# danielreardon/scintools

Measured on AMD Instinct MI355X. Metric: eta_curvature_sweep_points_per_sec, higher is better.
Workload: dtype f64

## Files before the change

scintools_amd/csrc/eigen_packed.hip:

```cpp
#include <math.h>
#include <string.h>

#include <algorithm>
#include <atomic>
#include <map>
#include <vector>

#include "packed.hpp"
#include "prof.hpp"

namespace scint {

constexpr int kCheckEveryBlock = 2;
constexpr int kFirstCheck = 8;
constexpr int kMaxK = 512;

__device__ inline cplx packed_at(const PackedJob& jb, int r, int c) {
    const int br = r / kTB, bc = c / kTB;
    if (bc >= br) return jb.tiles[(tile_offset(jb.nb, br) + (bc - br)) * kTileElems + (r % kTB) * kTB + (c % kTB)];
    return conj(jb.tiles[(tile_offset(jb.nb, bc) + (br - bc)) * kTileElems + (c % kTB) * kTB + (r % kTB)]);
}

constexpr int kRedGroups = 4;


__global__ void __launch_bounds__(64) pk_ritz_scale_kernel(const PackedJob* jobs, const int32_t* slots,
                                                           const int64_t* eta_index, cplx* vec_out,
                                                           int64_t vstride) {
    const PackedJob jb = jobs[slots[blockIdx.y]];
    const int K = blockIdx.x, e = threadIdx.x;
    if (K >= jb.nb) return;
    double t = 0.0;
    for (int i = e; i < jb.nb; i += 64) t += jb.upart[0][i];
    t = wave_sum(t);
    const double inv = t > 0.0 ? 1.0 / sqrt(t) : 0.0;
    const int r = K * kTB + e;
    cplx* out = vec_out + eta_index[blockIdx.y] * vstride;
    if (r < jb.n) out[r] = mk(out[r].x * inv, out[r].y * inv);
}

struct Blk2 {
    double a11, a22; cplx a12;
    double b11, b22; cplx b12;
    double i11, i22;
};

__device__ inline Blk2 step_block_wave(const double* __restrict__ ap, const double* __restrict__ up, int nb, int lane,
                                       bool direct = false) {
    double s[8];
#pragma unroll
    for (int c = 0; c < 8; ++c) s[c] = 0.0;
    for (int i = lane; i < nb; i += 64) {
#pragma unroll
        for (int c = 0; c < 4; ++c) { s[c] += gload(ap + 4 * i + c); s[4 + c] += gload(up + 4 * i + c); }
    }
#pragma unroll
    for (int c = 0; c < 8; ++c) s[c] = wave_sum(s[c]);
    Blk2 b;
    b.a11 = s[0]; b.a22 = s[1]; b.a12 = mk(s[2], s[3]);
    const double n12 = s[2] * s[2] + s[3] * s[3], tr = s[0] + s[1];
    const double h11 = direct ? s[4] : s[4] - (s[0] * s[0] + n12), h22 = direct ? s[5] : s[5] - (n12 + s[1] * s[1]);
    const cplx h12 = direct ? mk(s[6], s[7]) : mk(s[6] - s[2] * tr, s[7] - s[3] * tr);
    const double kPivotFloor = direct ? 0.0 : 1e-14;
    b.b11 = h11 > kPivotFloor * s[4] ? sqrt(h11) : 0.0;
    b.i11 = b.b11 > 0.0 ? 1.0 / b.b11 : 0.0;
    b.b12 = mk(h12.x * b.i11, h12.y * b.i11);
    const double d = h22 - norm2(b.b12);
    b.b22 = d > kPivotFloor * s[5] ? sqrt(d) : 0.0;
    b.i22 = b.b22 > 0.0 ? 1.0 / b.b22 : 0.0;
    return b;
}

__device__ inline void blk_q_row(const Blk2& b, cplx u1, cplx u2, cplx q1, cplx q2, cplx& x1, cplx& x2) {
    const cplx y1 = u1 - (q1 * b.a11 + mulc(q2, b.a12));
    const cplx y2 = u2 - (q1 * b.a12 + q2 * b.a22);
    x1 = y1 * b.i11;
    x2 = (y2 - x1 * b.b12) * b.i22;
}

__device__ inline int second_start_row(int n) { return (n / 2 + 7 < n) ? n / 2 + 7 : (n / 2 + 1) % max(n, 1); }

__global__ void __launch_bounds__(64) pk2_init_kernel(const PackedJob* jobs, const int32_t* slots) {
    const PackedJob jb = jobs[slots[blockIdx.y]];
    const int K = blockIdx.x, e = threadIdx.x;
    if (K == 0 && e == 0) { jb.state[1] = 0; jb.result[1] = -INFINITY; jb.result[3] = -INFINITY; }
    if (K >= jb.nb) return;
    const int r = K * kTB + e;
    cplx v0 = mk(0.0, 0.0), v1 = mk(0.0, 0.0);
    if (r < jb.n && jb.n >= 2) { v0 = packed_at(jb, jb.n / 2, r); v1 = packed_at(jb, second_start_row(jb.n), r); }
    jb.U[0][2 * r] = v0; jb.U[0][2 * r + 1] = v1;
    jb.U[1][2 * r] = mk(0.0, 0.0); jb.U[1][2 * r + 1] = mk(0.0, 0.0);
    cplx* qm1 = jb.Q + (int64_t)(jb.qslots - 1) * jb.qstride * 2;
    qm1[2 * r] = mk(0.0, 0.0); qm1[2 * r + 1] = mk(0.0, 0.0);
    jb.Q[2 * r] = mk(0.0, 0.0); jb.Q[2 * r + 1] = mk(0.0, 0.0);
    const double g11 = wave_sum(norm2(v0)), g22 = wave_sum(norm2(v1));
    const cplx g12 = wave_sum(mulc(v1, v0));
    if (e == 0) {
#pragma unroll
        for (int c = 0; c < 4; ++c) { jb.apart[0][4 * K + c] = 0.0; jb.apart[1][4 * K + c] = 0.0; jb.upart[1][4 * K + c] = 0.0; }
        jb.upart[0][4 * K] = g11; jb.upart[0][4 * K + 1] = g22; jb.upart[0][4 * K + 2] = g12.x; jb.upart[0][4 * K + 3] = g12.y;
    }
}

__device__ inline Blk2 load_blk(const double* __restrict__ c) {
    Blk2 b;
    b.a11 = gload(c + 0); b.a22 = gload(c + 1); b.a12 = mk(gload(c + 2), gload(c + 3));
    b.b11 = gload(c + 4); b.b22 = gload(c + 5); b.b12 = mk(gload(c + 6), gload(c + 7));
    b.i11 = gload(c + 8); b.i22 = gload(c + 9);
    return b;
}

constexpr int kCoefRows = 1024;
__global__ void __launch_bounds__(kCoefRows) pk2_coef_kernel(const PackedJob* __restrict__ jobs, int launch) {
    __shared__ double sh[16];
    const PackedJob jb = jobs[blockIdx.y];
    const int step = launch - jb.start;
    if (jb.n < 2 || step < 0 || step >= jb.max_steps || gload(jb.state) >= jb.gen) return;
    if ((int)blockIdx.x * kCoefRows >= jb.nb * kTB) return;
    const int par = step & 1;
    if (threadIdx.x < 64) {
        const Blk2 sc = step_block_wave(par ? jb.apart[1] : jb.apart[0], par ? jb.upart[1] : jb.upart[0], jb.nb, threadIdx.x,
                                        jb.certify && step == 1);
        if (threadIdx.x == 0) {
            sh[0] = sc.a11; sh[1] = sc.a22; sh[2] = sc.a12.x; sh[3] = sc.a12.y;
            sh[4] = sc.b11; sh[5] = sc.b22; sh[6] = sc.b12.x; sh[7] = sc.b12.y;
            sh[8] = sc.i11; sh[9] = sc.i22;
            if (blockIdx.x == 0) {
                double* c = jb.coef + 16 * par;
#pragma unroll
                for (int i = 0; i < 10; ++i) gstore(c + i, sh[i]);
                if (step > 0) {
                    double* A = jb.alpha + 4 * (step - 1);
                    A[0] = sc.a11; A[1] = sc.a22; A[2] = sc.a12.x; A[3] = sc.a12.y;
                }
                double* B = jb.beta + 4 * step;
                B[0] = sc.b11; B[1] = sc.b22; B[2] = sc.b12.x; B[3] = sc.b12.y;
            }
        }
    }
    __syncthreads();
    Blk2 sc;
    sc.a11 = sh[0]; sc.a22 = sh[1]; sc.a12 = mk(sh[2], sh[3]);
    sc.b11 = sh[4]; sc.b22 = sh[5]; sc.b12 = mk(sh[6], sh[7]);
    sc.i11 = sh[8]; sc.i22 = sh[9];
    const int r = (int)blockIdx.x * kCoefRows + (int)threadIdx.x;
    if (r >= jb.nb * kTB) return;
    const cplx* __restrict__ Up = par ? jb.U[1] : jb.U[0];
    const int qs = jb.qslots;
    const cplx* __restrict__ Qp = jb.Q + (int64_t)((step + qs - 1) % qs) * jb.qstride * 2;
    cplx* __restrict__ Qn = jb.Q + (int64_t)(step % qs) * jb.qstride * 2;
    cplx x1, x2;
    blk_q_row(sc, gload(Up + 2 * r), gload(Up + 2 * r + 1), gload(Qp + 2 * r), gload(Qp + 2 * r + 1), x1, x2);
    gstore(Qn + 2 * r, x1); gstore(Qn + 2 * r + 1, x2);
}

constexpr int kLdsXs = 0, kLdsCol = kMaxStrip * kTB * 2, kLdsXi = 2 * kLdsCol, kLdsRsum = kLdsXi + kRows64 * kTB * 2,
              kLdsElems = kLdsRsum + 4 * kTB * 2;
constexpr size_t kMatvecLdsBytes = sizeof(cplx) * kLdsElems;
static_assert(kMatvecLdsBytes <= 80 * 1024, "two mat-vec workgroups per CU (160 KiB of LDS)");

__device__ __forceinline__ void pk2_half(const cplx (&a)[8], int h, const cplx (*__restrict__ xir)[2],
                                        const cplx (&xJ1)[2], const cplx (&xJ2)[2], cplx (&acc1)[8], cplx (&acc2)[8],
                                        cplx (&c1)[2], cplx (&c2)[2]) {
#pragma unroll
    for (int jj = 0; jj < 4; ++jj) {
        const int j = 4 * h + jj;
        const cplx x1 = xir[8 * j][0], x2 = xir[8 * j][1];
#pragma unroll
        for (int cc = 0; cc < 2; ++cc) {
            const cplx e = a[2 * jj + cc];
            acc1[j] = acc1[j] + e * xJ1[cc];
            acc2[j] = acc2[j] + e * xJ2[cc];
            c1[cc] = mk(c1[cc].x + e.x * x1.x + e.y * x1.y, c1[cc].y + e.x * x1.y - e.y * x1.x);
            c2[cc] = mk(c2[cc].x + e.x * x2.x + e.y * x2.y, c2[cc].y + e.x * x2.y - e.y * x2.x);
        }
// ... 134 lines not shown

__global__ void __launch_bounds__(256, 2)
pk2_matvec_kernel(const Strip* __restrict__ strips, int launch) {
    pk2_matvec_body(strips + blockIdx.x, launch);
}

}
#include "matvec32.hpp"
namespace scint {

__global__ void __launch_bounds__(64 * kRedGroups)
pk2_reduce_kernel(const PackedJob* __restrict__ jobs, int launch) {
    __shared__ cplx part[kRedGroups][kTB][2];
    const PackedJob jb = jobs[blockIdx.y];
    const int K = blockIdx.x;
    const int step = launch - jb.start;
    if (K >= jb.nb || jb.n < 2 || step < 0 || step >= jb.max_steps || gload(jb.state) >= jb.gen) return;
    const int par = step & 1;
    const int g = threadIdx.x >> 6, e = threadIdx.x & 63;
    const int s0 = jb.row_strip0[K], nrow = jb.row_strip0[K + 1] - s0;
    cplx acc1 = mk(0.0, 0.0), acc2 = mk(0.0, 0.0);
    const int lg = jb.rowgroup_lg;
    const int npair = (K + (1 << lg) - 1) >> lg;
    for (int idx = g; idx < nrow + npair; idx += kRedGroups) {
        const int cI = (idx - nrow) << lg;
        const cplx* src = idx < nrow ? jb.rowpart + 2 * ((int64_t)(s0 + idx) * kTB + e)
                                     : jb.colpart + 2 * ((tile_offset(jb.nb, cI) + (K - cI)) * kTB + e);
        acc1 = acc1 + gload(src);
        acc2 = acc2 + gload(src + 1);
    }
    part[g][e][0] = acc1;
    part[g][e][1] = acc2;
    __syncthreads();
    if (g == 0) {
        const Blk2 sc = load_blk(jb.coef + 16 * par);
        cplx tot1 = part[0][e][0], tot2 = part[0][e][1];
#pragma unroll
        for (int k = 1; k < kRedGroups; ++k) { tot1 = tot1 + part[k][e][0]; tot2 = tot2 + part[k][e][1]; }
        const int r = K * kTB + e;
        const cplx* __restrict__ Qp = jb.Q + (int64_t)((step + jb.qslots - 1) % jb.qslots) * jb.qstride * 2;
        const cplx* __restrict__ Qn = jb.Q + (int64_t)(step % jb.qslots) * jb.qstride * 2;
        cplx* __restrict__ Un = par ? jb.U[0] : jb.U[1];
        const cplx q1 = gload(Qp + 2 * r), q2 = gload(Qp + 2 * r + 1);
        const cplx x1 = gload(Qn + 2 * r), x2 = gload(Qn + 2 * r + 1);
        const cplx t1 = tot1 - (q1 * sc.b11 + mulc(q2, sc.b12));
        const cplx t2 = tot2 - q2 * sc.b22;
        gstore(Un + 2 * r, t1); gstore(Un + 2 * r + 1, t2);
        const double pa11 = wave_sum(x1.x * t1.x + x1.y * t1.y);
        const double pa22 = wave_sum(x2.x * t2.x + x2.y * t2.y);
        const cplx pa12 = wave_sum(mulc(t2, x1));
        const double pg11 = wave_sum(norm2(t1)), pg22 = wave_sum(norm2(t2));
        const cplx pg12 = wave_sum(mulc(t2, t1));
        if (e == 0) {
            double* an = par ? jb.apart[0] : jb.apart[1];
            double* un = par ? jb.upart[0] : jb.upart[1];
            an[4 * K] = pa11; an[4 * K + 1] = pa22; an[4 * K + 2] = pa12.x; an[4 * K + 3] = pa12.y;
            un[4 * K] = pg11; un[4 * K + 1] = pg22; un[4 * K + 2] = pg12.x; un[4 * K + 3] = pg12.y;
        }
    }
}

__global__ void __launch_bounds__(64) pk2_cert_resid_kernel(const PackedJob* __restrict__ jobs, int launch) {
    const PackedJob jb = jobs[blockIdx.y];
    const int K = blockIdx.x, e = threadIdx.x;
    if (!jb.certify || launch - jb.start != 0 || K >= jb.nb || jb.n < 2 || gload(jb.state) >= jb.gen) return;
    const Blk2 sc = step_block_wave(jb.apart[1], jb.upart[1], jb.nb, e);
    const int r = K * kTB + e;
    const cplx* __restrict__ Q0 = jb.Q;
    const cplx u1 = gload(jb.U[1] + 2 * r), u2 = gload(jb.U[1] + 2 * r + 1);
    const cplx q1 = gload(Q0 + 2 * r), q2 = gload(Q0 + 2 * r + 1);
    const cplx y1 = u1 - (q1 * sc.a11 + mulc(q2, sc.a12));
    const cplx y2 = u2 - (q1 * sc.a12 + q2 * sc.a22);
    const double g11 = wave_sum(norm2(y1)), g22 = wave_sum(norm2(y2));
    const cplx g12 = wave_sum(mulc(y2, y1));
    if (e == 0) { double* un = jb.upart[1]; un[4 * K] = g11; un[4 * K + 1] = g22; un[4 * K + 2] = g12.x; un[4 * K + 3] = g12.y; }
}

constexpr int kMaxKB = 128;
constexpr int kSvecStride = 2 * kMaxKB + 4;

__device__ inline int band_count(const double* dg, const cplx* e1, const cplx* e2, int n, double x, double tiny) {
    int cnt = 0;
    double r1 = 0.0, r2 = 0.0;
    cplx p = mk(0.0, 0.0), q = mk(0.0, 0.0);
    for (int i = 0; i < n; ++i) {
        double d = ((dg[i] - x) - norm2(p) * r1) - norm2(q) * r2;
        if (fabs(d) < tiny) d = -tiny;
        cnt += d < 0.0;
        const cplx below = i >= 1 ? e2[i - 1] : mk(0.0, 0.0);
        const cplx pn = e1[i] - mulc(below, p) * r1;
        q = below;
        p = pn;
        r2 = r1;
        r1 = 1.0 / d;
    }
    return cnt;
}

__device__ inline double band_multisect(const double* dg, const cplx* e1, const cplx* e2, int n, int target,
                                        double lo, double hi, double tiny, int lane) {
    for (int round = 0; round < 48; ++round) {
        const double wdt = hi - lo;
        if (!(wdt > 0.0)) break;
        const double x = lo + wdt * ((double)(lane + 1) / 65.0);
        const int ok = (x > lo && x < hi) ? (band_count(dg, e1, e2, n, x, tiny) >= target) : 0;
        const unsigned long long m = __ballot(ok);
        double nlo, nhi;
        if (m == 0ull) { nlo = __shfl(x, 63, 64); nhi = hi; }
        else {
            const int first = __ffsll((long long)m) - 1;
            nhi = __shfl(x, first, 64);
            nlo = first > 0 ? __shfl(x, first - 1, 64) : lo;
        }
        if (!(nlo > lo) && !(nhi < hi)) break;
        if (nlo > lo) lo = nlo;
        if (nhi < hi) hi = nhi;
        if (hi - lo <= 2e-16 * fmax(fabs(lo), fabs(hi))) break;
    }
    return 0.5 * (lo + hi);
}

__global__ void __launch_bounds__(64) pk2_check_kernel(const PackedJob* jobs, int launches_done) {
    __shared__ double dg[2 * kMaxKB + 2];
    __shared__ cplx e1[2 * kMaxKB + 2], e2[2 * kMaxKB + 2];
    __shared__ double fd[2 * kMaxKB + 2];
    __shared__ cplx fm[2 * kMaxKB + 2];
    __shared__ cplx sv[2 * kMaxKB + 2];
    const PackedJob jb = jobs[blockIdx.x];
    if (jb.gen <= 0 || jb.state[0] >= jb.gen) return;
    const int lane = threadIdx.x;
    const int k_done = launches_done - jb.start;
    if (jb.n < 2) {
        if (lane == 0) {
            jb.state[2] = 0;
            jb.state[0] = jb.gen;
            jb.status_out[0] = SCINT_E_EMPTY;
            jb.eig_out[0] = nan("");
            if (jb.iters_out) jb.iters_out[0] = 0;
        }
        return;
    }
    if (k_done < kFirstCheck / 2 && k_done < jb.max_steps && !(jb.certify && k_done >= 1)) return;
    const int k = min(k_done, jb.max_steps);
    const int n = 2 * k;
    const Blk2 last = step_block_wave((k & 1) ? jb.apart[1] : jb.apart[0], (k & 1) ? jb.upart[1] : jb.upart[0], jb.nb, lane,
                                      jb.certify && k == 1);
    for (int j = lane; j < k; j += 64) {
        double a11, a22; cplx a12;
        if (j < k - 1) { const double* A = jb.alpha + 4 * j; a11 = A[0]; a22 = A[1]; a12 = mk(A[2], A[3]); }
        else { a11 = last.a11; a22 = last.a22; a12 = last.a12; }
        dg[2 * j] = a11; dg[2 * j + 1] = a22;
        e1[2 * j] = conj(a12);
        if (j + 1 < k) {
            const double* B = jb.beta + 4 * (j + 1);
            e2[2 * j] = mk(B[0], 0.0);
            e1[2 * j + 1] = mk(B[2], B[3]);
            e2[2 * j + 1] = mk(B[1], 0.0);
        } else {
            e2[2 * j] = mk(0.0, 0.0); e1[2 * j + 1] = mk(0.0, 0.0); e2[2 * j + 1] = mk(0.0, 0.0);
        }
    }
    __syncthreads();
    double lo = INFINITY, hi = -INFINITY, scale = 0.0;
    for (int i = lane; i < n; i += 64) {
        double off = 0.0;
        if (i >= 1) off += sqrt(norm2(e1[i - 1]));
        if (i >= 2) off += sqrt(norm2(e2[i - 2]));
        if (i + 1 < n) off += sqrt(norm2(e1[i]));
        if (i + 2 < n) off += sqrt(norm2(e2[i]));
        lo = fmin(lo, dg[i] - off);
        hi = fmax(hi, dg[i] + off);
        scale = fmax(scale, fabs(dg[i]) + off);
    }
    for (int o = 32; o > 0; o >>= 1) {
        lo = fmin(lo, __shfl_xor(lo, o, 64));
        hi = fmax(hi, __shfl_xor(hi, o, 64));
        scale = fmax(scale, __shfl_xor(scale, o, 64));
    }
    const double bnorm = sqrt(last.b11 * last.b11 + last.b22 * last.b22 + norm2(last.b12));
    const bool finite = isfinite(lo) && isfinite(hi) && isfinite(bnorm);
    double theta = nan(""), theta2 = -INFINITY, resid = nan(""), err = nan("");
    bool have_vectors = false;
    double tiny = 0.0;
    auto inverse_iteration = [&](double value) {
        const double sigma = value + 8e-16 * fmax(fabs(value), scale * 1e-3);
        double r1 = 0.0, r2 = 0.0;
        cplx p = mk(0.0, 0.0), q = mk(0.0, 0.0);
        for (int i = 0; i < n; ++i) {
            double d = ((dg[i] - sigma) - norm2(p) * r1) - norm2(q) * r2;
            if (fabs(d) < tiny) d = -tiny;
            const cplx below = i >= 1 ? e2[i - 1] : mk(0.0, 0.0);
            const cplx pn = e1[i] - mulc(below, p) * r1;
            fd[i] = d; fm[i] = pn;
            q = below; p = pn; r2 = r1; r1 = 1.0 / d;
        }
        for (int i = 0; i < n; ++i) sv[i] = mk(1.0, 0.0);
        double nrm = 1.0;
        for (int it = 0; it < 2; ++it) {
            for (int i = 0; i < n; ++i) {
// ... 47 lines not shown
        const double prev = jb.result[3];
        const double at = fmax(fabs(theta), 1e-300);
        const bool settled = (theta - prev) <= 1e3 * jb.tol * at || (jb.certify && k == 1);
        const bool exact = finite && (n >= jb.n || bnorm == 0.0);
        const double prev2 = jb.result[1], gap2 = theta - theta2;
        const bool gap_ok = gap2 > 0.0 && fabs(theta2 - prev2) <= 0.02 * gap2;
        const bool vec_ok = (resid <= jb.tol * at) || (gap_ok && settled && resid <= jb.vec_gap_factor * jb.tol * gap2);
        const bool ok = (jb.want_vec && !jb.use32) ? vec_ok : (err <= jb.tol * at && settled);
        const bool conv = finite && (ok || exact);
        const bool stop = conv || !finite || k >= jb.max_steps;
        jb.result[0] = theta; jb.result[1] = theta2; jb.result[2] = resid; jb.result[3] = theta;
        if (stop) {
            const bool hand_over = jb.use32 && conv && have_vectors && isfinite(theta);
            if (hand_over) {
                cplx* out = (cplx*)jb.svec + kSvecStride;
                if (n >= 2 && theta2 > -INFINITY) {
                    const double nrm = inverse_iteration(theta2);
                    const double inv = nrm > 0.0 && isfinite(nrm) ? 1.0 / sqrt(nrm) : 0.0;
                    for (int i = 0; i < n; ++i) out[i] = sv[i] * inv;
                } else {
                    for (int i = 0; i < n; ++i) out[i] = mk(0.0, 0.0);
                }
            }
            const double unscale = jb.use32 ? 1.0 / gload(jb.scale32) : 1.0;
            jb.state[1] = k;
            jb.state[2] = hand_over ? 1 : 0;
            __threadfence();
            jb.state[0] = jb.gen;
            if (!hand_over) {
                jb.eig_out[0] = (jb.want_vec ? theta : fabs(theta)) * unscale;
                if (jb.iters_out) jb.iters_out[0] = k + jb.iters_base;
                jb.status_out[0] = (!finite || !isfinite(theta)) ? SCINT_E_NONFINITE : (conv ? SCINT_OK : SCINT_E_NOCONV);
            }
        }
    }
}

__global__ void __launch_bounds__(64) pk2_ritz_kernel(const PackedJob* jobs, const int32_t* slots,
                                                      const int64_t* eta_index, cplx* vec_out, int64_t vstride) {
    const PackedJob jb = jobs[slots[blockIdx.y]];
    const int K = blockIdx.x, e = threadIdx.x;
    if (K >= jb.nb) return;
    const int k = jb.state[1];
    const int r = K * kTB + e;
    const cplx* __restrict__ sv = (const cplx*)jb.svec;
    cplx y = mk(0.0, 0.0);
    for (int j = 0; j < k; ++j) {
        const cplx* __restrict__ q = jb.Q + (int64_t)j * jb.qstride * 2 + 2 * r;
        y = (y + q[0] * sv[2 * j]) + q[1] * sv[2 * j + 1];
    }
    cplx* out = vec_out + eta_index[blockIdx.y] * vstride;
    if (r < jb.n) out[r] = y;
    const double p = wave_sum(r < jb.n ? norm2(y) : 0.0);
    if (e == 0) jb.upart[0][K] = p;
}

__global__ void __launch_bounds__(64) pk2_restart_kernel(const PackedJob* jobs, const int32_t* slots) {
    const PackedJob jb = jobs[slots[blockIdx.y]];
    const int K = blockIdx.x, e = threadIdx.x;
    if (K == 0 && e == 0) { jb.state[1] = 0; jb.result[1] = -INFINITY; jb.result[3] = -INFINITY; }
    if (K >= jb.nb) return;
    const int r = K * kTB + e;
    const int k = jb.iters_base;
    const cplx* __restrict__ s1 = (const cplx*)jb.svec;
    const cplx* __restrict__ s2 = s1 + kSvecStride;
    cplx y1 = mk(0.0, 0.0), y2 = mk(0.0, 0.0);
    for (int j = 0; j < k; ++j) {
        const cplx* __restrict__ q = jb.Q + (int64_t)j * jb.qstride * 2 + 2 * r;
        const cplx q0 = q[0], q1 = q[1];
        y1 = (y1 + q0 * s1[2 * j]) + q1 * s1[2 * j + 1];
        y2 = (y2 + q0 * s2[2 * j]) + q1 * s2[2 * j + 1];
    }
    if (r >= jb.n) { y1 = mk(0.0, 0.0); y2 = mk(0.0, 0.0); }
    jb.U[0][2 * r] = y1; jb.U[0][2 * r + 1] = y2;
    jb.U[1][2 * r] = mk(0.0, 0.0); jb.U[1][2 * r + 1] = mk(0.0, 0.0);
    cplx* qm1 = jb.Q + (int64_t)(jb.qslots - 1) * jb.qstride * 2;
    qm1[2 * r] = mk(0.0, 0.0); qm1[2 * r + 1] = mk(0.0, 0.0);
    jb.Q[2 * r] = mk(0.0, 0.0); jb.Q[2 * r + 1] = mk(0.0, 0.0);
    const double g11 = wave_sum(norm2(y1)), g22 = wave_sum(norm2(y2));
    const cplx g12 = wave_sum(mulc(y2, y1));
    if (e == 0) {
#pragma unroll
        for (int c = 0; c < 4; ++c) { jb.apart[0][4 * K + c] = 0.0; jb.apart[1][4 * K + c] = 0.0; jb.upart[1][4 * K + c] = 0.0; }
        jb.upart[0][4 * K] = g11; jb.upart[0][4 * K + 1] = g22; jb.upart[0][4 * K + 2] = g12.x; jb.upart[0][4 * K + 3] = g12.y;
    }
}

struct SlabLayout {
    size_t tiles, tiles32, U0, U1, Q, svec, rowpart, colpart, apart0, apart1, upart0, upart1,
        coef, alpha, beta, result, total;
    int qslots;
};

static int strip_len32_for(int nb) { return std::min(strip_len_for(nb), kMaxStrip32); }

static int max_strips(int nb) {
    const int S = strip_len_for(nb);
    int n = 0;
    for (int I = 0; I < nb; ++I) n += row_strip_count(nb, I, S, kRows64);
    return n;
}
static int max_strips32(int nb) {
    const int S = strip_len32_for(nb);
    int n = 0;
    for (int I = 0; I < nb; ++I) n += row_strip_count(nb, I, S, kRows32);
    return n;
}

static SlabLayout slab_layout(int nbmax, int max_steps, bool want_vec, bool mixed) {
    SlabLayout L;
    size_t off = 0;
    auto take = [&](size_t bytes) { off = align_up(off, 256); size_t o = off; off += bytes; return o; };
    int smax = 0;
    for (int nb = 1; nb <= nbmax; ++nb) smax = std::max(smax, std::max(max_strips(nb), mixed ? max_strips32(nb) : 0));
    L.tiles = take(sizeof(cplx) * (size_t)tile_count(nbmax) * kTileElems);
    L.tiles32 = mixed ? take(sizeof(c32) * (size_t)tile_count(nbmax) * kTileElems) : 0;
    const size_t bw = 2, sc = bw * bw;
    L.U0 = take(sizeof(cplx) * (size_t)nbmax * kTB * bw);
    L.U1 = take(sizeof(cplx) * (size_t)nbmax * kTB * bw);
    L.qslots = want_vec ? max_steps + 1 : (mixed ? std::min(max_steps, kMaxKB) + 1 : 2);
    L.Q = take(sizeof(cplx) * (size_t)nbmax * kTB * (size_t)L.qslots * bw);
    L.svec = take(sizeof(cplx) * (size_t)std::max<int64_t>(bw * (int64_t)(max_steps + 2), 2 * kSvecStride));
    L.rowpart = take(sizeof(cplx) * (size_t)smax * kTB * bw);
    L.colpart = take(sizeof(cplx) * (size_t)tile_count(nbmax) * kTB * bw);
    L.apart0 = take(sizeof(double) * (size_t)nbmax * sc);
    L.apart1 = take(sizeof(double) * (size_t)nbmax * sc);
    L.upart0 = take(sizeof(double) * (size_t)nbmax * sc);
    L.upart1 = take(sizeof(double) * (size_t)nbmax * sc);
    L.coef = take(sizeof(double) * 32);
    L.alpha = take(sizeof(double) * (size_t)(max_steps + 2) * sc);
    L.beta = take(sizeof(double) * (size_t)(max_steps + 3) * sc);
    L.result = take(sizeof(double) * 4);
    L.total = align_up(off, 256);
    return L;
}

constexpr int kTabs = 3;

struct BatchLayout {
    SlabLayout slab;
    int smax;
    size_t jobs, strips, strips32, states, slots, fin_slots, restart, fin_eta, rs, geoms, scales, scale_bits, total;
    size_t jobs_stride, strips_stride, strips32_stride, list_stride, fin_eta_stride, rs_stride;
};

static BatchLayout batch_layout(int nbmax, int max_steps, int nbatch, bool want_vec, int64_t ncs, bool mixed) {
    BatchLayout B;
    B.slab = slab_layout(nbmax, max_steps, want_vec, mixed);
    B.smax = 0;
    for (int nb = 1; nb <= nbmax; ++nb) B.smax = std::max(B.smax, std::max(max_strips(nb), mixed ? max_strips32(nb) : 0));
    size_t off = B.slab.total * (size_t)nbatch;
    auto take = [&](size_t bytes) { off = align_up(off, 256); size_t o = off; off += bytes; return o; };
    B.jobs_stride = align_up(sizeof(PackedJob) * (size_t)nbatch, 256);
    B.strips_stride = align_up(sizeof(Strip) * (size_t)nbatch * (size_t)B.smax, 256);
    B.strips32_stride = mixed ? align_up(sizeof(Strip32) * (size_t)nbatch * (size_t)B.smax, 256) : 0;
    B.list_stride = align_up(sizeof(int32_t) * (size_t)nbatch, 256);
    B.fin_eta_stride = align_up(sizeof(int64_t) * (size_t)nbatch, 256);
    B.jobs = take(B.jobs_stride * kTabs);
    B.strips = take(B.strips_stride * kTabs);
    B.strips32 = take(B.strips32_stride * kTabs);
    B.states = take(sizeof(int32_t) * 4 * (size_t)nbatch);
    B.slots = take(B.list_stride * kTabs);
    B.fin_slots = take(B.list_stride * kTabs);
    B.restart = take(B.list_stride * kTabs);
    B.fin_eta = take(B.fin_eta_stride * kTabs);
    B.rs_stride = align_up(sizeof(int32_t) * (size_t)nbatch * (size_t)(nbmax + 1), 256);
    B.rs = take(B.rs_stride * kTabs);
    B.geoms = take(sizeof(GeomDev) * (size_t)ncs);
    B.scales = take(sizeof(double) * (size_t)ncs);
    B.scale_bits = take(sizeof(unsigned long long) * (size_t)ncs);
    B.total = align_up(off, 256);
    return B;
}


static std::atomic<int>& sweep_mode_ref() {
    static std::atomic<int> mode([] {
        const char* e = getenv("SCINT_SWEEP_PRECISION");
        if (!e || !(e[0] == 'm' || e[0] == 'M')) return 0;
        return strncmp(e + 1, "ixed-all", 8) == 0 ? 2 : 1;
    }());
// ... 24 lines not shown
        auto env_int = [](const char* name) { const char* e = getenv(name); return e ? atoi(e) : 0; };
        sc.depth = env_int("SCINT_SWEEP_DEPTH"); sc.check_every = env_int("SCINT_CHECK_EVERY"); sc.groups = env_int("SCINT_SWEEP_GROUPS");
        return true;
    }();
    (void)init;
    return sc;
}

static char* pinned_staging(size_t bytes) {
    thread_local char* buf = nullptr;
    thread_local size_t cap = 0;
    if (bytes > cap) {
        if (buf) (void)hipHostFree(buf);
        buf = nullptr;
        cap = 0;
        const size_t want = std::max<size_t>(bytes + bytes / 4, 1 << 16);
        if (hipHostMalloc(&buf, want) != hipSuccess) {
            set_error("scint: hipHostMalloc of the sweep staging buffer failed");
            buf = nullptr;
            return nullptr;
        }
        cap = want;
    }
    return buf;
}

constexpr int kTabsEv = 3;
struct SideStreams {
    hipStream_t aux = nullptr, chk[2] = {}, tail[kTailLanes] = {};
    hipEvent_t chunk_done[2][kTabsEv] = {}, export_done[2][kTabsEv] = {}, steps_done[2][kTabsEv] = {};
    hipEvent_t start_ev = nullptr, stagger_ev = nullptr;
};
static SideStreams* side_streams() {
    thread_local std::map<int, SideStreams> streams;
    int dev = 0;
    if (hipGetDevice(&dev) != hipSuccess) return nullptr;
    auto it = streams.find(dev);
    if (it != streams.end()) return &it->second;
    SideStreams s;
    if (hipStreamCreateWithFlags(&s.aux, hipStreamNonBlocking) != hipSuccess) return nullptr;
    for (auto& c : s.chk)
        if (hipStreamCreateWithFlags(&c, hipStreamNonBlocking) != hipSuccess) return nullptr;
    for (auto& t : s.tail)
        if (hipStreamCreateWithFlags(&t, hipStreamNonBlocking) != hipSuccess) return nullptr;
    auto mk_ev = [](hipEvent_t* e) { return hipEventCreateWithFlags(e, hipEventDisableTiming) == hipSuccess; };
    for (int g = 0; g < 2; ++g)
        for (int t = 0; t < kTabsEv; ++t)
            if (!mk_ev(&s.chunk_done[g][t]) || !mk_ev(&s.export_done[g][t]) || !mk_ev(&s.steps_done[g][t])) return nullptr;
    if (!mk_ev(&s.start_ev) || !mk_ev(&s.stagger_ev)) return nullptr;
    return &(streams[dev] = s);
}

static_assert(kTabsEv == kTabs, "event sets per group = table copies");
struct SweepStats { double bytes32 = 0, bytes64 = 0, certified = 0, cert_passes = 0; };
static SweepStats& sweep_stats() { thread_local SweepStats st; return st; }

struct SweepProblem {
    const cplx* cs; int64_t cs_stride; const int32_t* cs_index; const double* th_cents; int64_t M;
    const int32_t* keep_idx; const int32_t* keep_n; const double* etas; int64_t neta;
    double* eigs_out; int32_t* status_out; int32_t* iters_out;
    bool want_vec; cplx* vec_out; int64_t vstride;
    SweepTail* tail_hook; hipStream_t tail[kTailLanes]; int tail_rr = 0;
    int nbmax, steps_cap, depth, check_every;
    bool mixed = false; double tol = 0.0; const double* scales_dev = nullptr;
    char* base; BatchLayout BL; const GeomDev* geoms_dev; int32_t* states_dev;
    int64_t next_eta = 0;
    hipEvent_t stagger_ev = nullptr;
};

struct SweepGroup {
    SweepProblem* P;
    int slot0, nslots;
    hipStream_t stream;
    hipStream_t check_stream;
    hipEvent_t chunk_done[kTabs], export_done[kTabs], steps_done[kTabs];
    PackedJob* h_jobs[kTabs]; Strip* h_strips[kTabs]; int32_t* h_fresh[kTabs]; int32_t* h_fin[kTabs];
    int64_t* h_fin_eta[kTabs]; int32_t* h_rs[kTabs]; int32_t* h_flags[kTabs];
    Strip32* h_strips32[kTabs]; int32_t* h_restart[kTabs];
    std::vector<PackedJob> jobs;
    std::vector<int64_t> slot_eta;
    std::vector<int32_t> slot_gen;
    std::vector<int32_t> fin_slots;
    std::vector<int64_t> fin_eta;
    std::vector<int8_t> slot_phase;
    std::vector<std::pair<int32_t, int32_t>> restart;
    int nstrips32 = 0;
    int active = 0, chunk = 0, seen = 0;
    bool finished = false;
    int tab_of_chunk[kTabs];
    int nstrips = 0, nb_run = 1;

    PackedJob* d_jobs(int t) const { return (PackedJob*)(P->base + P->BL.jobs + P->BL.jobs_stride * (size_t)t) + slot0; }
    Strip* d_strips(int t) const {
        return (Strip*)(P->base + P->BL.strips + P->BL.strips_stride * (size_t)t) + (size_t)slot0 * (size_t)P->BL.smax;
    }
    int32_t* d_fresh(int t) const { return (int32_t*)(P->base + P->BL.slots + P->BL.list_stride * (size_t)t) + slot0; }
    int32_t* d_fin(int t) const { return (int32_t*)(P->base + P->BL.fin_slots + P->BL.list_stride * (size_t)t) + slot0; }
    int32_t* d_restart(int t) const { return (int32_t*)(P->base + P->BL.restart + P->BL.list_stride * (size_t)t) + slot0; }
    Strip32* d_strips32(int t) const {
        return (Strip32*)(P->base + P->BL.strips32 + P->BL.strips32_stride * (size_t)t) + (size_t)slot0 * (size_t)P->BL.smax;
    }
    int32_t* d_rs(int t) const {
        return (int32_t*)(P->base + P->BL.rs + P->BL.rs_stride * (size_t)t) + (size_t)slot0 * (size_t)(P->nbmax + 1);
    }
    int64_t* d_fin_eta(int t) const { return (int64_t*)(P->base + P->BL.fin_eta + P->BL.fin_eta_stride * (size_t)t) + slot0; }

// ... 151 lines not shown
                for (size_t k = 0; k < fin_slots.size(); ++k) {
                    const PackedJob& F = h_jobs[ft][fin_slots[k]];
                    if (F.n < 2) continue;
                    h_fin[tab][nfin] = fin_slots[k];
                    h_fin_eta[tab][nfin] = fin_eta[k];
                    nb_fin = std::max(nb_fin, F.nb);
                    ++nfin;
                }
                if (nfin > 0) {
                    he = hipMemcpyAsync(d_fin(tab), h_fin[tab], sizeof(int32_t) * (size_t)nfin, hipMemcpyHostToDevice, stream);
                    if (he == hipSuccess)
                        he = hipMemcpyAsync(d_fin_eta(tab), h_fin_eta[tab], sizeof(int64_t) * (size_t)nfin,
                                            hipMemcpyHostToDevice, stream);
                    if (he != hipSuccess) return hip_fail(he, "sweep eigenvector export", __FILE__, __LINE__);
                    const dim3 grid((unsigned)nb_fin, (unsigned)nfin);
                    hipLaunchKernelGGL(pk2_ritz_kernel, grid, dim3(64), 0, stream, d_jobs(ft), d_fin(tab), d_fin_eta(tab),
                                       S.vec_out, S.vstride);
                    hipLaunchKernelGGL(pk_ritz_scale_kernel, grid, dim3(64), 0, stream, d_jobs(ft), d_fin(tab),
                                       d_fin_eta(tab), S.vec_out, S.vstride);
                }
            }
            if (S.tail_hook && !fin_eta.empty()) {
                he = hipEventRecord(export_done[tab], stream);
                for (int l = 0; l < kTailLanes && he == hipSuccess; ++l) he = hipStreamWaitEvent(S.tail[l], export_done[tab], 0);
                if (he != hipSuccess) return hip_fail(he, "sweep tail hand-off", __FILE__, __LINE__);
                const int bm = std::max(1, S.tail_hook->batch_max());
                for (size_t k0 = 0; k0 < fin_eta.size(); k0 += (size_t)bm) {
                    const int l = S.tail_rr++ % kTailLanes;
                    const int32_t rc = S.tail_hook->retire_batch(fin_eta.data() + k0, (int)std::min<size_t>((size_t)bm, fin_eta.size() - k0),
                                                                 S.tail[l], l);
                    if (rc != SCINT_OK) return rc;
                }
            }
            if (!restart.empty()) {
                int nb_re = 1;
                for (const auto& rs : restart) nb_re = std::max(nb_re, jobs[(size_t)rs.first].nb);
                hipLaunchKernelGGL(pk2_restart_kernel, dim3((unsigned)nb_re, (unsigned)restart.size()), dim3(64), 0, stream,
                                   d_jobs(tab), d_restart(tab));
            }
            if (!fresh.empty()) {
                int32_t rc = launch_gather_packed(S.geoms_dev, S.M, d_jobs(tab), d_fresh(tab), (int)fresh.size(), nb_fresh, stream,
                                                  S.mixed);
                if (rc != SCINT_OK) return rc;
                hipLaunchKernelGGL(pk2_init_kernel, dim3((unsigned)nb_fresh, (unsigned)fresh.size()), dim3(64), 0, stream,
                                   d_jobs(tab), d_fresh(tab));
            }
            he = hipGetLastError();
            if (he != hipSuccess) return hip_fail(he, "sweep refill", __FILE__, __LINE__);
        }
        tab_of_chunk[chunk % kTabs] = tab;
        if (nstrips + nstrips32 > 0) {
            for (int i = 0; i < S.check_every; ++i) {
                const int launch = launch0 + i;
                if (chunk > 0 && i == (S.check_every > 1 ? 1 : 0))
                    (void)hipStreamWaitEvent(stream, chunk_done[(chunk - 1) % kTabs], 0);
                hipLaunchKernelGGL(pk2_coef_kernel, dim3((unsigned)ceil_div(nb_run * kTB, kCoefRows), (unsigned)nslots),
                                   dim3(kCoefRows), 0, stream, d_jobs(tab), launch);
                if (nstrips32 > 0 && nstrips > 0) {
                    const int slot = profiler().begin(kProfMatvec32, stream);
                    hipLaunchKernelGGL(pk2_matvec_mixed_kernel, dim3((unsigned)(nstrips32 + nstrips)), dim3(256), kMatvecMixedLdsBytes, stream,
                                       d_strips32(tab), nstrips32, d_strips(tab), launch);
                    profiler().end(kProfMatvec32, slot, stream);
                } else if (nstrips32 > 0) {
                    const int slot = profiler().begin(kProfMatvec32, stream);
                    hipLaunchKernelGGL(pk2_matvec32_kernel, dim3((unsigned)nstrips32), dim3(256), kMatvec32LdsBytes, stream,
                                       d_strips32(tab), launch);
                    profiler().end(kProfMatvec32, slot, stream);
                } else if (nstrips > 0) {
                    const int slot = profiler().begin(kProfMatvec, stream);
                    hipLaunchKernelGGL(pk2_matvec_kernel, dim3((unsigned)nstrips), dim3(256), kMatvecLdsBytes, stream, d_strips(tab), launch);
                    profiler().end(kProfMatvec, slot, stream);
                }
                hipLaunchKernelGGL(pk2_reduce_kernel, dim3((unsigned)nb_run, (unsigned)nslots), dim3(64 * kRedGroups), 0,
                                   stream, d_jobs(tab), launch);
                if (!restart.empty() && i == S.check_every - 1)
                    hipLaunchKernelGGL(pk2_cert_resid_kernel, dim3((unsigned)nb_run, (unsigned)nslots), dim3(64), 0, stream,
                                       d_jobs(tab), launch);
                if (chunk == 0 && i == 0 && S.stagger_ev && slot0 == 0) (void)hipEventRecord(S.stagger_ev, stream);
            }
        }
        he = hipEventRecord(steps_done[chunk % kTabs], stream);
        if (he == hipSuccess) he = hipStreamWaitEvent(check_stream, steps_done[chunk % kTabs], 0);
        if (he != hipSuccess) return hip_fail(he, "sweep check hand-off", __FILE__, __LINE__);
        hipLaunchKernelGGL(pk2_check_kernel, dim3((unsigned)nslots), dim3(64), 0, check_stream, d_jobs(tab), launch0 + S.check_every);
        he = hipGetLastError();
        if (he == hipSuccess)
            he = hipMemcpyAsync(h_flags[chunk % kTabs], S.states_dev + 4 * slot0, sizeof(int32_t) * 4 * (size_t)nslots,
                                hipMemcpyDeviceToHost, check_stream);
        if (he == hipSuccess) he = hipEventRecord(chunk_done[chunk % kTabs], check_stream);
        if (he != hipSuccess) return hip_fail(he, "sweep chunk", __FILE__, __LINE__);
        ++chunk;
        return SCINT_OK;
    }

    int32_t advance() {
        SweepProblem& S = *P;
        int fin_chunk = -1;
        fin_slots.clear();
        fin_eta.clear();
        restart.clear();
        const bool more = active > 0 || S.next_eta < S.neta;
        if (chunk - seen >= S.depth || (!more && seen < chunk)) {
            hipError_t he = hipEventSynchronize(chunk_done[seen % kTabs]);
            if (he != hipSuccess) return hip_fail(he, "sweep wait", __FILE__, __LINE__);
            if (profiler().enabled) profiler().collect();
            harvest(seen);
            fin_chunk = seen++;
        }
// ... 72 lines not shown
        return align_up(sizeof(PackedJob) * nsl, 64) + align_up(sizeof(Strip) * nsl * (size_t)S.BL.smax, 64) +
               (S.mixed ? align_up(sizeof(Strip32) * nsl * (size_t)S.BL.smax, 64) : 0) +
               3 * align_up(sizeof(int32_t) * nsl, 64) + align_up(sizeof(int64_t) * nsl, 64) +
               align_up(sizeof(int32_t) * nsl * (size_t)(S.nbmax + 1), 64) + align_up(sizeof(int32_t) * 4 * nsl, 64);
    };
    const size_t geom_bytes = align_up(sizeof(GeomDev) * (size_t)ncs, 64);
    char* pin = pinned_staging(geom_bytes + per_tab((size_t)nslots) * kTabs + 64 * 9 * kTabs * 2);
    if (!pin) return SCINT_E_HIP;
    GeomDev* h_geoms = (GeomDev*)pin;
    for (int64_t c = 0; c < ncs; ++c) h_geoms[c] = to_dev(geom[c]);
    char* q = pin + geom_bytes;
    auto take = [&](size_t bytes) { char* r = q; q += align_up(bytes, 64); return r; };

    hipEvent_t start_ev = side->start_ev;
    hipError_t he = hipSuccess;
    int32_t rc = SCINT_OK;
    SweepGroup G[2];
    for (int g = 0; g < ngroups; ++g) {
        SweepGroup& grp = G[g];
        grp.P = &S;
        grp.slot0 = g == 0 ? 0 : nslots / 2;
        grp.nslots = (ngroups == 1 ? nslots : (g == 0 ? nslots / 2 : nslots - nslots / 2));
        grp.stream = g == 0 ? stream : side->aux;
        grp.check_stream = side->chk[g];
        const size_t nsl = (size_t)grp.nslots;
        for (int t = 0; t < kTabs; ++t) {
            grp.chunk_done[t] = side->chunk_done[g][t]; grp.export_done[t] = side->export_done[g][t];
            grp.steps_done[t] = side->steps_done[g][t];
            grp.h_jobs[t] = (PackedJob*)take(sizeof(PackedJob) * nsl);
            grp.h_strips[t] = (Strip*)take(sizeof(Strip) * nsl * (size_t)S.BL.smax);
            grp.h_fresh[t] = (int32_t*)take(sizeof(int32_t) * nsl);
            grp.h_fin[t] = (int32_t*)take(sizeof(int32_t) * nsl);
            grp.h_fin_eta[t] = (int64_t*)take(sizeof(int64_t) * nsl);
            grp.h_rs[t] = (int32_t*)take(sizeof(int32_t) * nsl * (size_t)(S.nbmax + 1));
            grp.h_flags[t] = (int32_t*)take(sizeof(int32_t) * 4 * nsl);
            grp.h_strips32[t] = (Strip32*)take(S.mixed ? sizeof(Strip32) * nsl * (size_t)S.BL.smax : 0);
            grp.h_restart[t] = (int32_t*)take(sizeof(int32_t) * nsl);
        }
        grp.jobs.assign(nsl, PackedJob());
        grp.slot_eta.assign(nsl, -1);
        grp.slot_gen.assign(nsl, 0);
        grp.slot_phase.assign(nsl, 0);
        for (int s = 0; s < grp.nslots; ++s) {
            char* sl = S.base + L.total * (size_t)(grp.slot0 + s);
            PackedJob& J = grp.jobs[(size_t)s];
            J.tiles = (cplx*)(sl + L.tiles);
            J.tiles32 = S.mixed ? (c32*)(sl + L.tiles32) : nullptr;
            J.scale32 = nullptr; J.use32 = 0; J.certify = 0; J.iters_base = 0; J.rowgroup_lg = kRows64Lg;
            J.U[0] = (cplx*)(sl + L.U0); J.U[1] = (cplx*)(sl + L.U1);
            J.Q = (cplx*)(sl + L.Q); J.qstride = (int64_t)S.nbmax * kTB; J.qslots = L.qslots;
            J.want_vec = want_vec ? 1 : 0; J.svec = (double*)(sl + L.svec);
            J.rowpart = (cplx*)(sl + L.rowpart); J.colpart = (cplx*)(sl + L.colpart);
            J.row_strip0 = nullptr;
            J.apart[0] = (double*)(sl + L.apart0); J.apart[1] = (double*)(sl + L.apart1);
            J.upart[0] = (double*)(sl + L.upart0); J.upart[1] = (double*)(sl + L.upart1);
            J.coef = (double*)(sl + L.coef);
            J.alpha = (double*)(sl + L.alpha); J.beta = (double*)(sl + L.beta);
            J.result = (double*)(sl + L.result); J.state = S.states_dev + 4 * (grp.slot0 + s);
            J.tol = tol; J.gen = 0;
            J.vec_gap_factor = tail_hook ? kVecGapFactorChisq : kVecGapFactor;
            J.n = 0; J.nb = 1; J.max_steps = 0; J.start = 0; J.strip_len = 1;
            J.eta = 0; J.two_eta = 0; J.keep = keep_idx;
            J.cs = (const cplx*)cs; J.th = th_cents; J.geom = 0; J.pad1 = 0;
            J.eig_out = eigs_out; J.status_out = status_out; J.iters_out = iters_out;
        }
    }
    if (rc == SCINT_OK) {
        he = hipMemcpyAsync((void*)S.geoms_dev, h_geoms, sizeof(GeomDev) * (size_t)ncs, hipMemcpyHostToDevice, stream);
        if (he == hipSuccess) he = hipMemsetAsync(S.states_dev, 0, sizeof(int32_t) * 4 * (size_t)nslots, stream);
        if (he == hipSuccess && S.mixed) {
            const int32_t src = launch_cs_scale((const cplx*)cs, ncs, cs_stride, (int64_t)geom[0].ntau * geom[0].nfd,
                                                (unsigned long long*)(S.base + S.BL.scale_bits), (double*)(S.base + S.BL.scales), stream);
            if (src != SCINT_OK) rc = src;
        }
        if (he == hipSuccess) he = hipMemsetAsync(status_out, 0x7f, sizeof(int32_t) * (size_t)neta, stream);
        if (he == hipSuccess && iters_out) he = hipMemsetAsync(iters_out, 0, sizeof(int32_t) * (size_t)neta, stream);
        if (he == hipSuccess && want_vec)
            he = hipMemsetAsync(vec_out, 0, sizeof(cplx) * (size_t)neta * (size_t)vstride, stream);
        if (he == hipSuccess) he = hipEventRecord(start_ev, stream);
        for (int l = 0; l < kTailLanes && he == hipSuccess; ++l) he = hipStreamWaitEvent(side->tail[l], start_ev, 0);
        if (he == hipSuccess) he = hipStreamWaitEvent(side->aux, start_ev, 0);
        if (he != hipSuccess) rc = hip_fail(he, "sweep setup", __FILE__, __LINE__);
    }
    if (rc == SCINT_OK && ngroups == 2) S.stagger_ev = side->stagger_ev;
    bool staggered = false;
    while (rc == SCINT_OK) {
        bool any = false;
        for (int g = 0; g < ngroups && rc == SCINT_OK; ++g) {
            if (G[g].finished) continue;
            any = true;
            if (g == 1 && !staggered) {
                staggered = true;
                if (G[0].chunk > 0 && G[0].nstrips + G[0].nstrips32 > 0) {
                    he = hipStreamWaitEvent(G[1].stream, S.stagger_ev, 0);
                    if (he != hipSuccess) { rc = hip_fail(he, "sweep stagger", __FILE__, __LINE__); break; }
                }
            }
            rc = G[g].advance();
        }
        if (!any) break;
    }
    hipError_t sync_err = hipStreamSynchronize(stream);
    { const hipError_t e2 = hipStreamSynchronize(side->aux); if (sync_err == hipSuccess) sync_err = e2; }
    for (auto& c : side->chk) { const hipError_t e2 = hipStreamSynchronize(c); if (sync_err == hipSuccess) sync_err = e2; }
    for (int l = 0; l < kTailLanes; ++l) {
        const hipError_t e2 = hipStreamSynchronize(side->tail[l]);
        if (sync_err == hipSuccess) sync_err = e2;
    }
// ... 109 lines not shown
```

scintools_amd/csrc/packed.hpp:

```cpp
#pragma once
#include <stdlib.h>

#include "thth.hpp"

namespace scint {

constexpr int kTB = 64;
constexpr int kTileElems = kTB * kTB;

struct __attribute__((aligned(8))) c32 { float x, y; };
static_assert(sizeof(c32) == 8, "c32 must be two floats");
#ifndef SCINT_ROWS32
#define SCINT_ROWS32 8
#endif
constexpr int kRows32 = SCINT_ROWS32;
constexpr int kRows32Lg = kRows32 == 8 ? 3 : (kRows32 == 4 ? 2 : (kRows32 == 2 ? 1 : 0));
static_assert((1 << kRows32Lg) == kRows32, "kRows32 must be 1, 2, 4 or 8");
#ifndef SCINT_MAXSTRIP32
#define SCINT_MAXSTRIP32 (SCINT_ROWS32 == 8 ? 12 : 14)
#endif
constexpr int kMaxStrip32 = SCINT_MAXSTRIP32;

__host__ __device__ inline int64_t tile_offset(int nb, int I) {
    return (int64_t)I * nb - (int64_t)I * (I - 1) / 2;
}
__host__ __device__ inline int64_t tile_count(int nb) { return (int64_t)nb * (nb + 1) / 2; }

#ifndef SCINT_ROWS64
#define SCINT_ROWS64 8
#endif
constexpr int kRows64 = SCINT_ROWS64;
constexpr int kRows64Lg = kRows64 == 16 ? 4 : (kRows64 == 8 ? 3 : (kRows64 == 4 ? 2 : 1));
static_assert(kRows64 == 2 || kRows64 == 4 || kRows64 == 8 || kRows64 == 16, "kRows64 must be 2, 4, 8 or 16");
#ifndef SCINT_MAXSTRIP
#define SCINT_MAXSTRIP (SCINT_ROWS64 == 8 ? 12 : (SCINT_ROWS64 == 4 ? 14 : (SCINT_ROWS64 == 16 ? 8 : 16)))
#endif
constexpr int kMaxStrip = SCINT_MAXSTRIP;
#ifndef SCINT_VEC_GAP_FACTOR
#define SCINT_VEC_GAP_FACTOR 30.0
#endif
#ifndef SCINT_VEC_GAP_FACTOR_CHISQ
#define SCINT_VEC_GAP_FACTOR_CHISQ 100.0
#endif
constexpr double kVecGapFactor = SCINT_VEC_GAP_FACTOR;
constexpr double kVecGapFactorChisq = SCINT_VEC_GAP_FACTOR_CHISQ;

inline int strip_len_for(int nb) {
    static const int forced = [] { const char* e = getenv("SCINT_STRIP_LEN"); return e ? atoi(e) : 0; }();
    if (forced > 0) return forced > kMaxStrip ? kMaxStrip : forced;
    return nb >= 16 ? kMaxStrip : (nb >= 8 ? 4 : (nb >= 4 ? 2 : 1));
}

struct PackedJob {
    double eta, two_eta;
    const cplx* cs;
    const double* th;
    int32_t geom, pad1;
    const int32_t* keep;
    int32_t n, nb;
    cplx* tiles;
    c32* tiles32;
    const double* scale32;
    int32_t use32;
    int32_t certify;
    int32_t iters_base;
    int32_t rowgroup_lg;
    int32_t max_steps, strip_len;
    int32_t start, gen;
    cplx* U[2];
    cplx* Q;
    int64_t qstride;
    int32_t qslots;
    int32_t want_vec;
    double* svec;
    cplx* rowpart;
    cplx* colpart;
    const int32_t* row_strip0;
    double* apart[2];
    double* upart[2];
    double* coef;
    double* alpha;
    double* beta;
    double* result;
    int32_t* state;
    double* eig_out; int32_t* status_out; int32_t* iters_out;
    double tol;
    double vec_gap_factor;
};

struct __attribute__((aligned(16))) Strip {
    const cplx* tiles[kRows64];
    cplx* rowpart[kRows64];
    const cplx* Q;
    cplx* colpart;
    const int32_t* state;
    int64_t qstride;
    int32_t I, J0, ntile, qslots;
    int32_t start, gen, max_steps, nrows;
};

inline int row_strip_count(int nb, int I, int S, int R) {
    const int lead = I - I % R;
    return (nb - lead + S - 1) / S;
}

struct __attribute__((aligned(16))) Strip32 {
    const c32* tiles[kRows32];
    cplx* rowpart[kRows32];
    const cplx* Q;
    cplx* colpart;
    const int32_t* state;
    int64_t qstride;
    int32_t I, J0, ntile, qslots;
    int32_t start, gen, max_steps, nrows;
};

int32_t launch_gather_packed(const GeomDev* geoms_dev, int64_t M, const PackedJob* jobs_dev,
                             const int32_t* slots_dev, int njobs, int nbmax, hipStream_t stream, bool with32 = false);
int32_t launch_cs_scale(const cplx* cs, int64_t ncs, int64_t cs_stride, int64_t nelem, unsigned long long* bits,
                        double* scale, hipStream_t stream);

#ifndef SCINT_TAIL_LANES
#define SCINT_TAIL_LANES 2
#endif
constexpr int kTailLanes = SCINT_TAIL_LANES;
struct SweepTail {
    virtual int32_t retire(int64_t eta_index, hipStream_t tail, int lane) = 0;
    virtual int32_t retire_batch(const int64_t* eta_index, int n, hipStream_t tail, int lane) {
        for (int k = 0; k < n; ++k) {
            const int32_t rc = retire(eta_index[k], tail, lane);
            if (rc != 0) return rc;
        }
// ... 18 lines not shown
```

Before: 1550.

## Use a three-entry ring for partial sums to defer cross-chunk event waits

Replaces the double-buffered apart/upart partial-sum arrays with a three-slot ring indexed by step modulo kSumRing, using a single base pointer plus stride. With the extra slot, the host no longer waits on the previous chunk's completion event at the second launch. It waits only when a launch would reuse a ring entry the convergence check may still read, which lets more kernel launches be queued ahead of the check. The cost is one more partial-sum buffer per slab and slightly more complex index arithmetic, plus some risk if the wait condition misses a dependency.

```diff
diff --git a/scintools_amd/csrc/eigen_packed.hip b/scintools_amd/csrc/eigen_packed.hip
--- a/scintools_amd/csrc/eigen_packed.hip
+++ b/scintools_amd/csrc/eigen_packed.hip
@@ -31,7 +31,7 @@
     const int K = blockIdx.x, e = threadIdx.x;
     if (K >= jb.nb) return;
     double t = 0.0;
-    for (int i = e; i < jb.nb; i += 64) t += jb.upart[0][i];
+    for (int i = e; i < jb.nb; i += 64) t += jb.upart[i];
     t = wave_sum(t);
     const double inv = t > 0.0 ? 1.0 / sqrt(t) : 0.0;
     const int r = K * kTB + e;
@@ -96,9 +96,10 @@
     const double g11 = wave_sum(norm2(v0)), g22 = wave_sum(norm2(v1));
     const cplx g12 = wave_sum(mulc(v1, v0));
     if (e == 0) {
-#pragma unroll
-        for (int c = 0; c < 4; ++c) { jb.apart[0][4 * K + c] = 0.0; jb.apart[1][4 * K + c] = 0.0; jb.upart[1][4 * K + c] = 0.0; }
-        jb.upart[0][4 * K] = g11; jb.upart[0][4 * K + 1] = g22; jb.upart[0][4 * K + 2] = g12.x; jb.upart[0][4 * K + 3] = g12.y;
+        double* a1 = jb.apart + jb.pstride; double* u1 = jb.upart + jb.pstride;
+#pragma unroll
+        for (int c = 0; c < 4; ++c) { jb.apart[4 * K + c] = 0.0; a1[4 * K + c] = 0.0; u1[4 * K + c] = 0.0; }
+        jb.upart[4 * K] = g11; jb.upart[4 * K + 1] = g22; jb.upart[4 * K + 2] = g12.x; jb.upart[4 * K + 3] = g12.y;
     }
 }
 
@@ -119,8 +120,8 @@
     if ((int)blockIdx.x * kCoefRows >= jb.nb * kTB) return;
     const int par = step & 1;
     if (threadIdx.x < 64) {
-        const Blk2 sc = step_block_wave(par ? jb.apart[1] : jb.apart[0], par ? jb.upart[1] : jb.upart[0], jb.nb, threadIdx.x,
-                                        jb.certify && step == 1);
+        const int64_t ring = sum_ring_entry(step) * jb.pstride;
+        const Blk2 sc = step_block_wave(jb.apart + ring, jb.upart + ring, jb.nb, threadIdx.x, jb.certify && step == 1);
         if (threadIdx.x == 0) {
             sh[0] = sc.a11; sh[1] = sc.a22; sh[2] = sc.a12.x; sh[3] = sc.a12.y;
             sh[4] = sc.b11; sh[5] = sc.b22; sh[6] = sc.b12.x; sh[7] = sc.b12.y;
@@ -361,8 +362,9 @@
         const double pg11 = wave_sum(norm2(t1)), pg22 = wave_sum(norm2(t2));
         const cplx pg12 = wave_sum(mulc(t2, t1));
         if (e == 0) {
-            double* an = par ? jb.apart[0] : jb.apart[1];
-            double* un = par ? jb.upart[0] : jb.upart[1];
+            const int64_t ring = sum_ring_entry(step + 1) * jb.pstride;
+            double* an = jb.apart + ring;
+            double* un = jb.upart + ring;
             an[4 * K] = pa11; an[4 * K + 1] = pa22; an[4 * K + 2] = pa12.x; an[4 * K + 3] = pa12.y;
             un[4 * K] = pg11; un[4 * K + 1] = pg22; un[4 * K + 2] = pg12.x; un[4 * K + 3] = pg12.y;
         }
@@ -373,7 +375,8 @@
     const PackedJob jb = jobs[blockIdx.y];
     const int K = blockIdx.x, e = threadIdx.x;
     if (!jb.certify || launch - jb.start != 0 || K >= jb.nb || jb.n < 2 || gload(jb.state) >= jb.gen) return;
-    const Blk2 sc = step_block_wave(jb.apart[1], jb.upart[1], jb.nb, e);
+    const int64_t ring = sum_ring_entry(1) * jb.pstride;
+    const Blk2 sc = step_block_wave(jb.apart + ring, jb.upart + ring, jb.nb, e);
     const int r = K * kTB + e;
     const cplx* __restrict__ Q0 = jb.Q;
     const cplx u1 = gload(jb.U[1] + 2 * r), u2 = gload(jb.U[1] + 2 * r + 1);
@@ -382,7 +385,7 @@
     const cplx y2 = u2 - (q1 * sc.a12 + q2 * sc.a22);
     const double g11 = wave_sum(norm2(y1)), g22 = wave_sum(norm2(y2));
     const cplx g12 = wave_sum(mulc(y2, y1));
-    if (e == 0) { double* un = jb.upart[1]; un[4 * K] = g11; un[4 * K + 1] = g22; un[4 * K + 2] = g12.x; un[4 * K + 3] = g12.y; }
+    if (e == 0) { double* un = jb.upart + ring; un[4 * K] = g11; un[4 * K + 1] = g22; un[4 * K + 2] = g12.x; un[4 * K + 3] = g12.y; }
 }
 
 constexpr int kMaxKB = 128;
@@ -452,8 +455,8 @@
     if (k_done < kFirstCheck / 2 && k_done < jb.max_steps && !(jb.certify && k_done >= 1)) return;
     const int k = min(k_done, jb.max_steps);
     const int n = 2 * k;
-    const Blk2 last = step_block_wave((k & 1) ? jb.apart[1] : jb.apart[0], (k & 1) ? jb.upart[1] : jb.upart[0], jb.nb, lane,
-                                      jb.certify && k == 1);
+    const int64_t ring = sum_ring_entry(k) * jb.pstride;
+    const Blk2 last = step_block_wave(jb.apart + ring, jb.upart + ring, jb.nb, lane, jb.certify && k == 1);
     for (int j = lane; j < k; j += 64) {
         double a11, a22; cplx a12;
         if (j < k - 1) { const double* A = jb.alpha + 4 * j; a11 = A[0]; a22 = A[1]; a12 = mk(A[2], A[3]); }
@@ -607,7 +610,7 @@
     cplx* out = vec_out + eta_index[blockIdx.y] * vstride;
     if (r < jb.n) out[r] = y;
     const double p = wave_sum(r < jb.n ? norm2(y) : 0.0);
-    if (e == 0) jb.upart[0][K] = p;
+    if (e == 0) jb.upart[K] = p;
 }
 
 __global__ void __launch_bounds__(64) pk2_restart_kernel(const PackedJob* jobs, const int32_t* slots) {
@@ -635,14 +638,15 @@
     const double g11 = wave_sum(norm2(y1)), g22 = wave_sum(norm2(y2));
     const cplx g12 = wave_sum(mulc(y2, y1));
     if (e == 0) {
-#pragma unroll
-        for (int c = 0; c < 4; ++c) { jb.apart[0][4 * K + c] = 0.0; jb.apart[1][4 * K + c] = 0.0; jb.upart[1][4 * K + c] = 0.0; }
-        jb.upart[0][4 * K] = g11; jb.upart[0][4 * K + 1] = g22; jb.upart[0][4 * K + 2] = g12.x; jb.upart[0][4 * K + 3] = g12.y;
+        double* a1 = jb.apart + jb.pstride; double* u1 = jb.upart + jb.pstride;
+#pragma unroll
+        for (int c = 0; c < 4; ++c) { jb.apart[4 * K + c] = 0.0; a1[4 * K + c] = 0.0; u1[4 * K + c] = 0.0; }
+        jb.upart[4 * K] = g11; jb.upart[4 * K + 1] = g22; jb.upart[4 * K + 2] = g12.x; jb.upart[4 * K + 3] = g12.y;
     }
 }
 
 struct SlabLayout {
-    size_t tiles, tiles32, U0, U1, Q, svec, rowpart, colpart, apart0, apart1, upart0, upart1,
+    size_t tiles, tiles32, U0, U1, Q, svec, rowpart, colpart, apart, upart, psum_stride,
         coef, alpha, beta, result, total;
     int qslots;
 };
@@ -678,10 +682,9 @@
     L.svec = take(sizeof(cplx) * (size_t)std::max<int64_t>(bw * (int64_t)(max_steps + 2), 2 * kSvecStride));
     L.rowpart = take(sizeof(cplx) * (size_t)smax * kTB * bw);
     L.colpart = take(sizeof(cplx) * (size_t)tile_count(nbmax) * kTB * bw);
-    L.apart0 = take(sizeof(double) * (size_t)nbmax * sc);
-    L.apart1 = take(sizeof(double) * (size_t)nbmax * sc);
-    L.upart0 = take(sizeof(double) * (size_t)nbmax * sc);
-    L.upart1 = take(sizeof(double) * (size_t)nbmax * sc);
+    L.psum_stride = align_up(sizeof(double) * (size_t)nbmax * sc, 256) / sizeof(double);
+    L.apart = take(sizeof(double) * L.psum_stride * kSumRing);
+    L.upart = take(sizeof(double) * L.psum_stride * kSumRing);
     L.coef = take(sizeof(double) * 32);
     L.alpha = take(sizeof(double) * (size_t)(max_steps + 2) * sc);
     L.beta = take(sizeof(double) * (size_t)(max_steps + 3) * sc);
@@ -812,6 +815,7 @@
 }
 
 static_assert(kTabsEv == kTabs, "event sets per group = table copies");
+static_assert(kSumRing >= 3 && kSumRing <= kTabs, "a check is waited for through the event set of a chunk at most kSumRing back");
 struct SweepStats { double bytes32 = 0, bytes64 = 0, certified = 0, cert_passes = 0; };
 static SweepStats& sweep_stats() { thread_local SweepStats st; return st; }
 
@@ -1069,8 +1073,9 @@
         if (nstrips + nstrips32 > 0) {
             for (int i = 0; i < S.check_every; ++i) {
                 const int launch = launch0 + i;
-                if (chunk > 0 && i == (S.check_every > 1 ? 1 : 0))
-                    (void)hipStreamWaitEvent(stream, chunk_done[(chunk - 1) % kTabs], 0);
+                const int seen_by = launch + 1 - kSumRing;
+                if (seen_by >= S.check_every && seen_by % S.check_every == 0)
+                    (void)hipStreamWaitEvent(stream, chunk_done[(seen_by / S.check_every - 1) % kTabs], 0);
                 hipLaunchKernelGGL(pk2_coef_kernel, dim3((unsigned)ceil_div(nb_run * kTB, kCoefRows), (unsigned)nslots),
                                    dim3(kCoefRows), 0, stream, d_jobs(tab), launch);
                 if (nstrips32 > 0 && nstrips > 0) {
@@ -1249,8 +1254,7 @@
             J.want_vec = want_vec ? 1 : 0; J.svec = (double*)(sl + L.svec);
             J.rowpart = (cplx*)(sl + L.rowpart); J.colpart = (cplx*)(sl + L.colpart);
             J.row_strip0 = nullptr;
-            J.apart[0] = (double*)(sl + L.apart0); J.apart[1] = (double*)(sl + L.apart1);
-            J.upart[0] = (double*)(sl + L.upart0); J.upart[1] = (double*)(sl + L.upart1);
+            J.apart = (double*)(sl + L.apart); J.upart = (double*)(sl + L.upart); J.pstride = (int64_t)L.psum_stride;
             J.coef = (double*)(sl + L.coef);
             J.alpha = (double*)(sl + L.alpha); J.beta = (double*)(sl + L.beta);
             J.result = (double*)(sl + L.result); J.state = S.states_dev + 4 * (grp.slot0 + s);
diff --git a/scintools_amd/csrc/packed.hpp b/scintools_amd/csrc/packed.hpp
--- a/scintools_amd/csrc/packed.hpp
+++ b/scintools_amd/csrc/packed.hpp
@@ -51,6 +51,9 @@
     return nb >= 16 ? kMaxStrip : (nb >= 8 ? 4 : (nb >= 4 ? 2 : 1));
 }
 
+constexpr int kSumRing = 3;
+__host__ __device__ inline int sum_ring_entry(int step) { return step % kSumRing; }
+
 struct PackedJob {
     double eta, two_eta;
     const cplx* cs;
@@ -76,8 +79,9 @@
     cplx* rowpart;
     cplx* colpart;
     const int32_t* row_strip0;
-    double* apart[2];
-    double* upart[2];
+    double* apart;
+    double* upart;
+    int64_t pstride;
     double* coef;
     double* alpha;
     double* beta;
```

After: 1544. Within noise of the previous version (-0.4%).
